# insitro/FastVim

Hardware: AMD Instinct MI355X
Metric: images/sec FastVim-T 224px bs=128/GPU fwd+bwd (+all-reduce +AdamW +EMA), whole job (higher is better)
Workload: dtype bf16; 1 GPU; FastVim-T 224x224 bs=128/GPU bf16 training step, synthetic ImageNet tensors (BASELINE configs[1]); global_batch=128, parallelism=dp1, hip_graph=True, optimizer_in_step=True, final_loss_hex=0x1.779ca20000000p+0

## Files before the change

### fastvim_amd/_lib.py

```python
import ctypes
import os
import threading

import torch

_PKG = os.path.dirname(os.path.abspath(__file__))
LIB_PATH = os.path.join(_PKG, "libfastvim_hip.so")

FV_F32, FV_BF16, FV_F16 = 0, 1, 2
_DTYPES = {torch.float32: FV_F32, torch.bfloat16: FV_BF16, torch.float16: FV_F16}

_lib = None

C_ABI_SYMBOLS = (
    "fv_last_error", "fv_version",
    "fv_selective_scan_fwd", "fv_selective_scan_bwd_workspace", "fv_selective_scan_bwd",
    "fv_causal_conv1d_fwd", "fv_causal_conv1d_bwd", "fv_scan_expand_skip_fwd",
    "fv_mixer_conv_pool_fwd", "fv_mixer_scan_fwd", "fv_mixer_xproj_scan_fwd_ok", "fv_mixer_xproj_scan_fwd", "fv_mixer_combine_fwd",
    "fv_mixer_bwd_blocks", "fv_mixer_combine_bwd", "fv_mixer_scan_bwd_chunks", "fv_mixer_scan_bwd_chunks_b",
    "fv_mixer_scan_bwd_ckpt_floats", "fv_mixer_scan_bwd_partials", "fv_mixer_scan_bwd", "fv_mixer_scan_bwd_dir", "fv_mixer_scan_bwd_ckpt", "fv_mixer_scan_bwd_segments", "fv_mixer_scan_bwd_seg_floats", "fv_mixer_scan_bwd_seg_partials", "fv_mixer_scan_bwd_seg_chunks", "fv_mixer_scan_bwd_seg", "fv_mixer_scan_fwd_ckpt", "fv_mixer_scan_ckpt_floats", "fv_mixer_scan_fwd_segments", "fv_mixer_scan_fwd_seg_floats", "fv_mixer_scan_fwd_seg", "fv_rows_segment_sum", "fv_rows_gather", "fv_mixer_conv_pool_bwd", "fv_mixer_conv_pool_bwd2_ok", "fv_mixer_conv_pool_bwd2", "fv_mixer_scan_bwd_xproj_ok", "fv_mixer_scan_bwd_xproj", "fv_chunk_rows_bf16", "fv_reduce_partials", "fv_reduce_partials_multi",
    "fv_add_norm_blocks", "fv_add_norm_fwd", "fv_add_norm_bwd", "fv_gemm_bf16", "fv_gemm_bf16_tn_grouped", "fv_gemm_bf16_tn_grouped_ld", "fv_mixer_xproj_fwd", "fv_mixer_xproj_bwd_slices", "fv_mixer_xproj_bwd", "fv_mixer_xproj_bwd2", "fv_mixer_xproj_bwd3_ok", "fv_mixer_xproj_bwd3", "fv_adamw_flat", "fv_soft_target_ce",
    "fv_patch_unfold", "fv_gemm_bf16_rowbias", "fv_mean_pool_fwd", "fv_mean_pool_bwd", "fv_droppath_table", "fv_scale_cast",
    "fv_column_sum", "fv_gemm_bf16_addnorm", "fv_gemm_bf16_dgrad_addnorm_blocks", "fv_gemm_bf16_dgrad_addnorm_bwd", "fv_gemm_bf16_dgrad_addnorm_bwd2", "fv_gemm_bf16_addnorm2", "fv_mixer_combine_out_proj_addnorm_ok", "fv_mixer_combine_out_proj_addnorm", "fv_gemm_f32",
    "fv_mixer_conv_pool_bwd_dgrad_ok", "fv_mixer_conv_pool_bwd_dgrad_blocks", "fv_mixer_conv_pool_bwd_dgrad", "fv_transpose_bf16_batched", "fv_gemm_bf16_tn_grouped_wide8",
    "fv_grad_sumsq_blocks", "fv_grad_sumsq_partials", "fv_adamw_flat_groups",
    "fv_pack_weight_frags_batched", "fv_mixer_conv_pool_bwd_dgrad_pk", "fv_mixer_combine_out_proj_addnorm_pk",
    "fv_mix_batch", "fv_patch_unfold_mix", "fv_mixup_target", "fv_label_ce",
    "fv_patch_unfold_chan", "fv_chan_embed_table", "fv_chan_embed_scatter",
)


_tls = threading.local()


class _DeviceGuarded:

    def __init__(self, cdll):
        self._cdll = cdll
        self._wrapped = {}

    def __getattr__(self, name):
        w = self._wrapped.get(name)
        if w is None:
            fn = getattr(self._cdll, name)

            def call(*args, _fn=fn):
                dev = getattr(_tls, "dev", None)
                if dev is None or dev == torch.cuda.current_device():
                    return _fn(*args)
                with torch.cuda.device(dev):
                    return _fn(*args)

            w = self._wrapped[name] = call
        return w


def lib():
    global _lib
    if _lib is None:
        if not os.path.exists(LIB_PATH):
            raise RuntimeError(
                f"{LIB_PATH} is missing: build it with `python -m fastvim_amd.build` "
                "(or __graft_entry__.build()). fastvim_amd has no CPU / eager fallback.")
        cdll = ctypes.CDLL(LIB_PATH)
        cdll.fv_last_error.restype = ctypes.c_char_p
        cdll.fv_selective_scan_bwd_workspace.restype = ctypes.c_size_t
        cdll.fv_mixer_scan_bwd_ckpt_floats.restype = ctypes.c_size_t
        cdll.fv_mixer_scan_ckpt_floats.restype = ctypes.c_size_t
        cdll.fv_mixer_scan_fwd_seg_floats.restype = ctypes.c_size_t
        cdll.fv_mixer_scan_bwd_seg_floats.restype = ctypes.c_size_t
        _lib = _DeviceGuarded(cdll)
    return _lib


def dtype_code(dt):
    try:
        return _DTYPES[dt]
    except KeyError:
        raise RuntimeError(f"fastvim_amd: unsupported dtype {dt}") from None
# ... 26 lines not shown
```

### fastvim_amd/csrc/combine_gemm.hip

```cpp
#include "mixer_common.h"
#include "packed.h"

namespace {

typedef __bf16 cg_bf16x8 __attribute__((ext_vector_type(8)));
typedef float cg_f32x4 __attribute__((ext_vector_type(4)));

constexpr int CG_K = 384, CG_N = 192, CG_BM = 64, CG_NT = 256;
constexpr int CG_RSA = CG_K * 2 + 16;
constexpr int CG_RSB = CG_N * 2 + 16;
constexpr int CG_PD = 6;
constexpr int CG_KS = CG_K / 32;
#ifndef CG_FORCE_PK
#define CG_FORCE_PK 0
#endif
#ifndef CG_DBG
#define CG_DBG 0
#endif

struct CgParams {
  const void* xz;
  const void* skip;
  const float* yc;
  const float *lnw, *lnb;
  void* g;
  float *mean, *rstd_ln;
  float ln_eps;
  Geo geo;
  int B;
  const bf16_t* W;
  long ldw;
  const float* residual;
  const float* nw;
  const float* row_scale;
  int rows_per_scale;
  float* res_out;
  bf16_t* y;
  float* rstd;
  float eps;
  int M;
  int d_in;
};

__device__ __forceinline__ float cg_hsum(f2 v) { return v.x + v.y; }

template <bool PK>
__global__ __launch_bounds__(CG_NT, 2) void combine_out_proj_addnorm_kernel(CgParams p) {
  extern __shared__ __attribute__((aligned(16))) char smem[];
  typedef PairVec<bf16_t, 3> P;
  const int tid = threadIdx.x, lane = tid & 63;
  const int wv = __builtin_amdgcn_readfirstlane(tid >> 6);
  const Geo g = p.geo;
  const int tiles = (g.rows + 3) / 4;
  const int bimg = blockIdx.x / tiles, i0 = (blockIdx.x - bimg * tiles) * 4;
  const int mimg = bimg * g.L;
  auto tok_of = [&](int rl) {
    const int w = rl >> 4, j = rl & 15;
    return (i0 + w < g.rows && j < g.cols) ? mimg + (i0 + w) * g.s_i + j * g.s_j : -1;
  };

  const int lr = lane % 16, gr = lane / 16;
  const int fn = lane & 15, fk = lane >> 4;
  const bf16_t* wrow[3];
  cg_bf16x8 fb[CG_PD][3];
  const char* wpk = reinterpret_cast<const char*>(p.W) + wv * (CG_KS * 3 * 1024);
  const uint32_t wpk_lane = (uint32_t)lane * 16;
  auto wfrag = [&](int nb, int ks) {
    if constexpr (PK) return *reinterpret_cast<const cg_bf16x8*>(wpk + (ks * 3 + nb) * 1024 + wpk_lane);
    else return *reinterpret_cast<const cg_bf16x8*>(wrow[nb] + ks * 32);
  };
  float4 ne_r[2][2][3], ne_w[3];
  float ne_sc[2][2];
  {
#pragma clang fp reassociate(off) contract(off)
    const int lc = lane * 6, voff = lc * 2;
    const int tok_x = 2 * CG_K * 2, tok_s = CG_K * 2;
    const bool has_ln = p.lnw != nullptr;
    const float inv_d = 1.f / (float)p.d_in;
    const size_t ydir = (size_t)p.B * g.rows * CG_K;
    const __amdgpu_buffer_rsrc_t bz = fv_make_buf((const bf16_t*)p.xz + CG_K, (size_t)p.M * tok_x - tok_s);
    const __amdgpu_buffer_rsrc_t bs = fv_make_buf(p.skip, (size_t)p.M * tok_s);
    const __amdgpu_buffer_rsrc_t bg = fv_make_buf(p.g, (size_t)p.M * tok_s);
    const __amdgpu_buffer_rsrc_t bmean = fv_make_buf(has_ln ? (const void*)p.mean : p.g, has_ln ? (size_t)p.M * 4 : 0);
    const __amdgpu_buffer_rsrc_t brstd = fv_make_buf(has_ln ? (const void*)p.rstd_ln : p.g, has_ln ? (size_t)p.M * 4 : 0);
    const int irow = i0 + wv;
    const bool wlive = irow < g.rows;
    const int irc = wlive ? irow : g.rows - 1;
    const int mbase = mimg + irc * g.s_i;
    char* arow = smem + (wv * 16) * CG_RSA + lane * 12;
    constexpr int TT = 2;
    const int npair = (g.cols + TT - 1) / TT;
    f2 ysum[3], ysf[3], ysb[3];
    {
      const float* yr = p.yc + ((size_t)bimg * g.rows + irc) * CG_K + lc;
#pragma unroll
      for (int q = 0; q < 3; ++q) {
        ysf[q] = *reinterpret_cast<const f2*>(yr + 2 * q);
        ysb[q] = *reinterpret_cast<const f2*>(yr + ydir + 2 * q);
      }
    }
    struct Pre { P sk[TT], z[TT]; };
    Pre pa, pb;
    auto fetch = [&](Pre& r, int j0) {
#pragma unroll
      for (int t = 0; t < TT; ++t) {
        const int m = mbase + min(j0 + t, g.cols - 1) * g.s_j;
        r.sk[t].load(bs, voff, m * tok_s);
        r.z[t].load(bz, voff, m * tok_x);
      }
    };
    fetch(pa, 0);
    fetch(pb, TT);
    __builtin_amdgcn_sched_barrier(0);
    f2 lw[3], lb[3];
    {
      const float* lwp = has_ln ? p.lnw : p.yc;
      const float* lbp = has_ln ? p.lnb : p.yc;
#pragma unroll
      for (int q = 0; q < 3; ++q) {
        lw[q] = *reinterpret_cast<const f2*>(lwp + lc + 2 * q);
        lb[q] = *reinterpret_cast<const f2*>(lbp + lc + 2 * q);
      }
    }
    __builtin_amdgcn_sched_barrier(0);
#pragma unroll
    for (int nb = 0; nb < 3; ++nb) wrow[nb] = PK ? nullptr : p.W + (long)(wv * 48 + nb * 16 + fn) * p.ldw + fk * 8;
#pragma unroll
    for (int s = 0; s < CG_PD; s += 2)
#pragma unroll
      for (int nb = 0; nb < 3; ++nb)
#pragma unroll
        for (int h = 0; h < 2; ++h) fb[s + h][nb] = wfrag(nb, s + h);
    __builtin_amdgcn_sched_barrier(0);
#pragma unroll
    for (int q = 0; q < 3; ++q) ysum[q] = ysf[q] + ysb[q];
    auto process = [&](Pre& r, int j0) {
      f2 o[TT][3], z[TT][3];
      float s1[TT], mean[TT], rstd[TT];
#pragma unroll
// ... 184 lines not shown
      for (int k = 0; k < 3; ++k) {
        const int c = (k * LPR + lr) * 4;
        float o[4];
#pragma unroll
        for (int e = 0; e < 4; ++e) {
          float t = v[u][k][e] * rstd;
          asm volatile("" : "+v"(t));
          o[e] = t * w[k][e];
        }
        uint2 pk = {pack_bf16x2(o[0], o[1]), pack_bf16x2(o[2], o[3])};
        if (live) *reinterpret_cast<uint2*>(p.y + base + c) = pk;
      }
    }
  }
}

}

extern "C" int fv_mixer_combine_out_proj_addnorm_ok(int batch, int rows, int cols, int tokens_per_patch, int d_inner,
                                                    int d_model, int dtype) {
  return dtype == FV_BF16 && d_inner == CG_K && d_model == CG_N && tokens_per_patch == 1 && batch > 0 && rows > 0 &&
         cols > 0 && cols <= 16 && (long)batch * rows * cols * CG_K * 4 < 0x7fffffffL;
}

static int cg_launch(bool packed, const void* xz, const void* skip, const float* yc, const float* ln_w,
                                                 const float* ln_b, float ln_eps, void* g, float* mean, float* rstd_ln,
                                                 int batch, int rows, int cols, int tok_stride_row, int tok_stride_col,
                                                 const void* W, long ldw, const float* residual,
                                                 const float* norm_weight, const float* row_scale, int rows_per_scale,
                                                 void* y, float* residual_out, float* rstd, float eps,
                                                 fv_stream_t stream) {
  FV_CHECK(xz && skip && yc && g && W && residual && norm_weight && y && residual_out && rstd,
           "mixer_combine_out_proj_addnorm: null pointer");
  FV_CHECK(!ln_w || (ln_b && mean && rstd_ln), "mixer_combine_out_proj_addnorm: LayerNorm needs weight, bias, mean, rstd");
  FV_CHECK(fv_mixer_combine_out_proj_addnorm_ok(batch, rows, cols, 1, CG_K, CG_N, FV_BF16),
           "mixer_combine_out_proj_addnorm: shape not built (fv_mixer_combine_out_proj_addnorm_ok)");
  FV_CHECK((tok_stride_row == cols && tok_stride_col == 1) || (tok_stride_row == 1 && tok_stride_col == rows),
           "mixer_combine_out_proj_addnorm: token strides (%d,%d) are neither row-major nor transposed for a %dx%d grid",
           tok_stride_row, tok_stride_col, rows, cols);
  FV_CHECK(((uintptr_t)W & 15) == 0 && ldw % 8 == 0 && ldw >= CG_K, "mixer_combine_out_proj_addnorm: weight rows must be 16-byte aligned");
  FV_CHECK(!packed || ldw == CG_K, "mixer_combine_out_proj_addnorm_pk: the packed weight has no row padding (ldw = %d)", CG_K);
  FV_CHECK(((uintptr_t)residual & 15) == 0 && ((uintptr_t)residual_out & 15) == 0 && ((uintptr_t)y & 7) == 0 &&
               ((uintptr_t)norm_weight & 15) == 0, "mixer_combine_out_proj_addnorm: row operands must be 16-byte aligned");
  FV_CHECK(!row_scale || rows_per_scale > 0, "mixer_combine_out_proj_addnorm: rows_per_scale must be positive");
  CgParams p{};
  p.xz = xz; p.skip = skip; p.yc = yc; p.lnw = ln_w; p.lnb = ln_b; p.g = g; p.mean = mean; p.rstd_ln = rstd_ln;
  p.ln_eps = ln_eps;
  p.geo = make_geo(rows, cols, tok_stride_row, tok_stride_col, 1);
  p.B = batch;
  p.W = (const bf16_t*)W; p.ldw = ldw; p.residual = residual; p.nw = norm_weight; p.row_scale = row_scale;
  p.rows_per_scale = rows_per_scale; p.res_out = residual_out; p.y = (bf16_t*)y; p.rstd = rstd; p.eps = eps;
  p.M = batch * rows * cols;
  p.d_in = CG_K;
  const size_t smem = (size_t)CG_BM * CG_RSA;
  const dim3 grid(batch * fv_cdiv(rows, 4)), block(CG_NT);
  if (packed || CG_FORCE_PK) hipLaunchKernelGGL(combine_out_proj_addnorm_kernel<true>, grid, block, smem, (hipStream_t)stream, p);
  else hipLaunchKernelGGL(combine_out_proj_addnorm_kernel<false>, grid, block, smem, (hipStream_t)stream, p);
  FV_LAUNCH_CHECK();
  return FV_OK;
}

#define CG_ARGS_DECL                                                                                                          \
  const void *xz, const void *skip, const float *yc, const float *ln_w, const float *ln_b, float ln_eps, void *g,             \
      float *mean, float *rstd_ln, int batch, int rows, int cols, int tok_stride_row, int tok_stride_col, const void *W,      \
      long ldw, const float *residual, const float *norm_weight, const float *row_scale, int rows_per_scale, void *y,         \
      float *residual_out, float *rstd, float eps, fv_stream_t stream
#define CG_ARGS                                                                                                               \
  xz, skip, yc, ln_w, ln_b, ln_eps, g, mean, rstd_ln, batch, rows, cols, tok_stride_row, tok_stride_col, W, ldw, residual,    \
      norm_weight, row_scale, rows_per_scale, y, residual_out, rstd, eps, stream

extern "C" int fv_mixer_combine_out_proj_addnorm(CG_ARGS_DECL) { return cg_launch(false, CG_ARGS); }

extern "C" int fv_mixer_combine_out_proj_addnorm_pk(CG_ARGS_DECL) { return cg_launch(true, CG_ARGS); }
```

### fastvim_amd/csrc/convpool_dgrad.hip

```cpp
#include "mixer_common.h"
#include "packed.h"
#include "gemm_tiles.h"

namespace {

constexpr int CD_DI = 384, CD_N = 192, CD_K = 2 * CD_DI, CD_BM = 64, CD_NT = 256, CD_NCH = CD_DI / 128;
constexpr int CD_RSA = CD_DI * 2 + 16;
constexpr int CD_RSB = CD_N * 2 + 16;
#ifndef CD_PDEPTH
#define CD_PDEPTH 4
#endif
#ifndef CD_SB_EVERY
#define CD_SB_EVERY 1
#endif
#ifndef CD_W2_PIPE
#define CD_W2_PIPE 1
#endif
constexpr int CD_PD = CD_PDEPTH;
constexpr int CD_KS = CD_K / 32;
constexpr int CD_ZST = CD_BM * BK * 2;
constexpr int CD_NZ = CD_DI / BK;
constexpr int CD_O_RING = CD_BM * CD_RSA;
constexpr int CD_SLOT = 12 * 128;
constexpr int CD_O_B = (CD_BM * CD_RSB + 255) / 256 * 256, CD_O_S = CD_O_B + 2 * 128 * BK * 2;
constexpr int CD_SMEM = CD_O_S + 4 * 32 * (64 * 2 + 16);
static_assert(CD_O_RING + 3 * CD_ZST <= CD_SMEM && CD_O_RING + 4 * CD_SLOT * 4 <= CD_SMEM, "LDS regions");
static_assert(2 * CD_SMEM <= 160 * 1024, "two workgroups per CU");
#ifndef CD_FORCE_PK
#define CD_FORCE_PK 0
#endif
#ifndef CD_DBG
#define CD_DBG 0
#endif

struct CdParams {
  const void* xz;
  const void* dob;
  const float* dxc;
  const void* dxc2;
  const float *wf, *bf, *wb, *bb, *Df, *Db;
  void* dxz;
  float* part;
  float pool_scale;
  Geo geo;
  int B;
  const bf16_t* Wt;
  long ldwt;
  const float* dres_out;
  const float* r;
  const float* rstd;
  const float* nw;
  const float* row_scale;
  int rows_per_scale;
  bf16_t* dx;
  float* dres_in;
  float* pw;
  const bf16_t* W2;
  long ldw2;
  bf16_t* C2;
  int N2;
  int M;
};

__device__ __forceinline__ void cd_dma16(const void* base, uint32_t voff, uint32_t lds_dst) {
  asm volatile("s_mov_b32 m0, %2\n\ts_nop 0\n\tglobal_load_lds_dwordx4 %0, %1" ::"v"(voff), "s"(base), "s"(lds_dst) : "memory");
}

constexpr int cd_younger(int t) {
  constexpr int KX = CD_DI / 32;
  int n = 0;
  for (int q = KX + 2 * (t - 3) + 2; q < KX + 2 * t; q += 2) n += (q + CD_PD < CD_KS ? 6 : 0) + ((q - KX) / 2 + 3 < CD_NZ ? 2 : 0);
  return n;
}
static_assert(cd_younger(3) < 64 && cd_younger(4) < 64 && cd_younger(5) < 64, "vmcnt is a 6-bit counter");

template <int NT, bool X2, bool PK>
__global__ __launch_bounds__(CD_NT, 2) void conv_pool_bwd_dgrad_kernel(CdParams p) {
  extern __shared__ __attribute__((aligned(16))) char smem[];
  typedef PairVec<bf16_t, 1> P;
  const int tid = threadIdx.x, lane = tid & 63;
  const int wv = __builtin_amdgcn_readfirstlane(tid >> 6);
  const Geo g = p.geo;
  const int tiles = (g.rows + 3) / 4;
  const int bimg = blockIdx.x / tiles, i0 = (blockIdx.x - bimg * tiles) * 4;
  const int mimg = bimg * g.L;
  auto tok_of = [&](int rl) {
    const int w = rl >> 4, j = rl & 15;
    return (i0 + w < g.rows && j < g.cols) ? mimg + (i0 + w) * g.s_i + j * g.s_j : -1;
  };
  const int irow = i0 + wv;
  const bool wlive = irow < g.rows;
  char* prow = smem + (wv * 16) * CD_RSA;

  {
    const int zr0 = wlive ? NT : 0;
    for (int e = lane; e < (16 - zr0) * (CD_RSA / 4); e += 64) reinterpret_cast<uint32_t*>(prow + zr0 * CD_RSA)[e] = 0u;
    const int tok_x = 2 * CD_DI * 2, tok_d = CD_DI * 2;
    const size_t dstride = (size_t)p.B * g.rows * CD_DI;
    const __amdgpu_buffer_rsrc_t bp = fv_make_buf(p.dxc, 2 * dstride * 4);
    const __amdgpu_buffer_rsrc_t bp2 = fv_make_buf(X2 ? p.dxc2 : p.dxc, X2 ? 2 * dstride * 2 : 0);
    const int irc = wlive ? irow : 0;
    const bool up = irc > 0, down = irc + 1 < g.rows;
    const int m_row = irc * g.s_i, s_up = up ? -g.s_i : 0, s_dn = down ? g.s_i : 0;
    const int pooled_off = (bimg * g.rows + irc) * CD_DI;
    const size_t img_x = (size_t)bimg * g.L * 2 * CD_DI, img_d = (size_t)bimg * g.L * CD_DI;
    const __amdgpu_buffer_rsrc_t bx = fv_make_buf((const bf16_t*)p.xz + img_x, wlive ? (size_t)g.L * tok_x : 0);
    const __amdgpu_buffer_rsrc_t bd = fv_make_buf((const bf16_t*)p.dob + img_d, wlive ? (size_t)g.L * tok_d : 0);
    const __amdgpu_buffer_rsrc_t bo = fv_make_buf((bf16_t*)p.dxz + img_x, wlive ? (size_t)g.L * tok_x : 0);
    struct Pooled {
      f2 a;
      P b;
      __device__ __forceinline__ f2 sum() const { if constexpr (X2) return a + b.get(0); else return a; }
    };
    auto pooled = [&](int r, bool backward, int c0, bool on) {
      const bool ok = r == 1 || (r == 0 ? up : down);
      uint32_t w[2];
      const int eoff = pooled_off + (ok ? (r - 1) * CD_DI : 0) + (backward ? (int)dstride : 0);
      const int lane_off = on ? c0 : 0x1ffffff0;
      fv_buf_load_words<2>(bp, lane_off * 4, eoff * 4, w);
      Pooled o;
      o.a.x = __uint_as_float(w[0]);
      o.a.y = __uint_as_float(w[1]);
      if constexpr (X2) o.b.load(bp2, lane_off * 2, eoff * 2);
      return o;
    };
    P xr[NT + 6], dr[NT + 6];
    auto fetch = [&](int k, int voff) {
      const int di = k < 3 ? -1 : (k >= NT + 3 ? 1 : 0);
      const int j = k - 3 - di * NT;
      const int m = m_row + (di < 0 ? s_up : di > 0 ? s_dn : 0) + j * g.s_j;
      xr[k].load(bx, voff, m * tok_x);
      dr[k].load(bd, voff, m * tok_d);
    };
    struct Prm { f2 wf[CW], wb[CW], bf, bb, Df, Db; };
    auto load_prm = [&](int c0) {
      Prm q;
      load_taps2(p.wf, c0, q.wf);
      load_taps2(p.wb, c0, q.wb);
      q.bf = load_f2(p.bf ? p.bf : p.wf, c0);
      q.bb = load_f2(p.bb ? p.bb : p.wf, c0);
      q.Df = load_f2(p.Df ? p.Df : p.wf, c0);
      q.Db = load_f2(p.Db ? p.Db : p.wf, c0);
      return q;
    };
// ... 51 lines not shown
            pf = fma2(wf[k], x[k0 + k], pf);
            pb = fma2(wb[k], x[k3 - k], pb);
          }
          const f2 sgf = sigmoid2(pf), sgb = sigmoid2(pb);
          const f2 dsf = sgf * fma2(pf, 1.f - sgf, splat(1.f)), dsb = sgb * fma2(pb, 1.f - sgb, splat(1.f));
          const float e3 = q3 < NT ? 1.f : m_dn, e0 = n >= 0 ? 1.f : m_up;
          if (q3 == NT) cf_dn = cf_dn_raw.sum() * (down ? p.pool_scale : 0.f);
          const f2 nf = fma2(Dfh, dov[k3], q3 >= NT ? cf_dn : cf_mid) * dsf * e3;
          const f2 nb = fma2(Dbh, dov[k0], n < 0 ? cb_up : cb_mid) * dsb * e0;
          if (n == -1) cb_up_raw = pooled(0, true, c0n, more);
          dpf[k3] = nf;
          dpb[k0] = nb;
          if (q3 < NT) {
#pragma unroll
            for (int k = 0; k < CW; ++k) a_wf[k] = fma2(nf, x[k0 + k], a_wf[k]);
            a_bf += nf;
            a_Df = fma2(dov[k3], pf * sgf, a_Df);
          }
          if (n >= 0) {
#pragma unroll
            for (int k = 0; k < CW; ++k) a_wb[k] = fma2(nb, x[k3 - k], a_wb[k]);
            a_bb += nb;
            a_Db = fma2(dov[k0], pb * sgb, a_Db);
            f2 dx = splat(0.f);
#pragma unroll
            for (int k = 0; k < CW; ++k) {
              dx = fma2(wf[k], dpf[k3 - k], dx);
              dx = fma2(wb[k], dpb[k0 - 3 + k], dx);
            }
            const uint32_t pk[1] = {pack_bf16x2(dx.x, dx.y)};
            fv_buf_store_words<1>(bo, voff, (m_row + n * g.s_j) * tok_x, pk);
            *reinterpret_cast<uint32_t*>(prow + n * CD_RSA + voff) = pk[0];
          }
          if ((n + 3) % CD_SB_EVERY == CD_SB_EVERY - 1) __builtin_amdgcn_sched_barrier(0);
        }
        cf_dn_raw = pooled(2, false, c0n, more);
      }
      {
        const f2 hDf = a_Df * 0.5f, hDb = a_Db * 0.5f;
        float4* s4 = reinterpret_cast<float4*>(slot);
        s4[2 * lane] = make_float4(a_wf[0].x, a_wf[1].x, a_wf[2].x, a_wf[3].x);
        s4[2 * lane + 1] = make_float4(a_wf[0].y, a_wf[1].y, a_wf[2].y, a_wf[3].y);
        s4[128 + 2 * lane] = make_float4(a_wb[0].x, a_wb[1].x, a_wb[2].x, a_wb[3].x);
        s4[128 + 2 * lane + 1] = make_float4(a_wb[0].y, a_wb[1].y, a_wb[2].y, a_wb[3].y);
        f2* s2 = reinterpret_cast<f2*>(slot + 1024);
        s2[lane] = a_bf;
        s2[64 + lane] = a_bb;
        s2[128 + lane] = hDf;
        s2[192 + lane] = hDb;
      }
      __syncthreads();
      {
        const float* s0 = reinterpret_cast<const float*>(smem + CD_O_RING);
        float* dst = p.part + (size_t)blockIdx.x * 12 * CD_DI;
#pragma unroll
        for (int i = 0; i < CD_SLOT / CD_NT; ++i) {
          const int e = tid + i * CD_NT;
          const float v = ((s0[e] + s0[CD_SLOT + e]) + s0[2 * CD_SLOT + e]) + s0[3 * CD_SLOT + e];
          int gi;
          if (e < 512) gi = c * 512 + e;
          else if (e < 1024) gi = 4 * CD_DI + c * 512 + (e - 512);
          else {
            const int q = (e - 1024) >> 7, rr = (e - 1024) & 127;
            gi = (8 + q) * CD_DI + c * 128 + rr;
          }
          dst[gi] = v;
        }
      }
      __syncthreads();
    }
  }

  const int fn = lane & 15, fk = lane >> 4, lr = lane % 16, gr = lane / 16;
  const bf16_t* wrow[3];
  bf16x8 fb[CD_PD][3];
#pragma unroll
  for (int nb = 0; nb < 3; ++nb) wrow[nb] = PK ? nullptr : p.Wt + (long)(wv * 48 + nb * 16 + fn) * p.ldwt + fk * 8;
  const char* wpk = reinterpret_cast<const char*>(p.Wt) + wv * (CD_KS * 3 * 1024);
  const uint32_t wpk_lane = (uint32_t)lane * 16;
  auto wfrag = [&](int nb, int ks) {
    if constexpr (PK) return *reinterpret_cast<const bf16x8*>(wpk + (ks * 3 + nb) * 1024 + wpk_lane);
    else return *reinterpret_cast<const bf16x8*>(wrow[nb] + ks * 32);
  };
  uint32_t zoff[2];
  const uint32_t ring = (uint32_t)(uintptr_t)(__attribute__((address_space(3))) const char*)(smem + CD_O_RING);
#pragma unroll
  for (int i = 0; i < 2; ++i) {
    const int e = tid + i * CD_NT, rrow = e >> 3, ch = (e & 7) ^ (rrow & 7);
    const int m = tok_of(rrow);
    zoff[i] = (uint32_t)((m >= 0 ? m : mimg) * (CD_K * 2) + (CD_DI + ch * 8) * 2);
  }
  auto issue_z = [&](int t) {
#pragma unroll
    for (int i = 0; i < 2; ++i)
      cd_dma16(p.dxz, zoff[i] + (uint32_t)t * (BK * 2), ring + (uint32_t)(t % 3) * CD_ZST + (uint32_t)(i * CD_NT + wv * 64) * 16);
  };
  issue_z(0);
  issue_z(1);
  issue_z(2);
#pragma unroll
  for (int s = 0; s < CD_PD; s += 2)
#pragma unroll
    for (int nb = 0; nb < 3; ++nb)
#pragma unroll
      for (int h = 0; h < 2; ++h) fb[s + h][nb] = wfrag(nb, s + h);
  __builtin_amdgcn_sched_barrier(0);
  float4 ne_r[2][2][3];
// ... 121 lines not shown
#pragma unroll
          for (int e = 0; e < 4; ++e) {
            const float dyl = dyv[e] * lv;
            xh[k][e] = (rr[e] - 0.f) * rstd;
            dxh[k][e] = dyl * w[k][e];
            aw[k][e] = fmaf(dyl, xh[k][e], aw[k][e]);
            c2 = fmaf(dxh[k][e], xh[k][e], c2);
          }
        }
#define FV_DPP_ADD(ctrl) c2 += __int_as_float(__builtin_amdgcn_update_dpp(0, __float_as_int(c2), ctrl, 0xf, 0xf, true))
        FV_DPP_ADD(0xB1);
        FV_DPP_ADD(0x4E);
        FV_DPP_ADD(0x141);
        FV_DPP_ADD(0x140);
#undef FV_DPP_ADD
        c2 = c2 * inv_n;
        const float c1 = 0.f;
#pragma unroll
        for (int k = 0; k < 3; ++k) {
          const int c = (k * LPR + lr) * 4;
          const float4 g4 = ne_g[it][u][k];
          const float gg[4] = {g4.x, g4.y, g4.z, g4.w};
          float dr[4];
#pragma unroll
          for (int e = 0; e < 4; ++e) dr[e] = rstd * (dxh[k][e] - c1 - xh[k][e] * c2) + gg[e];
          if (live) {
            *reinterpret_cast<float4*>(p.dres_in + base + c) = make_float4(dr[0], dr[1], dr[2], dr[3]);
            if (p.row_scale)
#pragma unroll
              for (int e = 0; e < 4; ++e) dr[e] *= sc;
            uint2 pk = {pack_bf16x2(dr[0], dr[1]), pack_bf16x2(dr[2], dr[3])};
            *reinterpret_cast<uint2*>(p.dx + base + c) = pk;
            *reinterpret_cast<uint2*>(smem + rl * CD_RSB + c * 2) = pk;
          } else {
            *reinterpret_cast<uint2*>(smem + rl * CD_RSB + c * 2) = make_uint2(0u, 0u);
          }
        }
      }
    }
    __syncthreads();
    float* s_acc = reinterpret_cast<float*>(smem + CD_BM * CD_RSB);
#pragma unroll
    for (int k = 0; k < 3; ++k)
#pragma unroll
      for (int e = 0; e < 4; ++e) {
        float v = aw[k][e];
        auto r1 = __builtin_amdgcn_permlane16_swap(__float_as_uint(v), __float_as_uint(v), false, false);
        v = __uint_as_float(r1[0]) + __uint_as_float(r1[1]);
        auto r2 = __builtin_amdgcn_permlane32_swap(__float_as_uint(v), __float_as_uint(v), false, false);
        v = __uint_as_float(r2[0]) + __uint_as_float(r2[1]);
        if (gr == 0) s_acc[wv * CD_N + (k * LPR + lr) * 4 + e] = v;
      }
    __syncthreads();
    float* dst = p.pw + (size_t)blockIdx.x * CD_N;
    for (int c = tid; c < CD_N; c += CD_NT) dst[c] = (s_acc[c] + s_acc[CD_N + c]) + (s_acc[2 * CD_N + c] + s_acc[3 * CD_N + c]);
  }
  if (p.W2 && CD_DBG != 4) {
    __syncthreads();
    tile_times_w2_rows<CD_BM, CD_RSB, KS, decltype(tok_of), CD_W2_PIPE != 0>(smem, smem + CD_O_B, smem + CD_O_S, p.W2, p.ldw2, p.N2,
                                                                              p.C2, tok_of, tid);
  }
}

}

extern "C" int fv_mixer_conv_pool_bwd_dgrad_ok(int batch, int rows, int cols, int tokens_per_patch, int d_inner, int d_model,
                                               int pool_max, int dtype) {
  return dtype == FV_BF16 && d_inner == CD_DI && d_model == CD_N && tokens_per_patch == 1 && !pool_max && batch > 0 &&
         rows > 0 && (cols == 14 || cols == 16) &&
         (long)batch * rows * cols * CD_K * 2 < 0x7fffffffL &&
         (long)batch * rows * CD_DI * 8 < 0x7ffff000L;
}

extern "C" int fv_mixer_conv_pool_bwd_dgrad_blocks(int batch, int rows) { return batch * fv_cdiv(rows, 4); }

static int cd_launch(
    bool packed, const void* xz, const void* dskip, const float* dxc, const void* dxc2, const float* conv_w, const float* conv_b,
    const float* conv_w_b, const float* conv_b_b, const float* D, const float* D_b, void* dxz, float* conv_partials, int batch,
    int rows, int cols, int tok_stride_row, int tok_stride_col, float scaling, const void* W_in_t, long ldwt,
    const float* dresidual_out, const float* r, const float* rstd, const float* norm_weight, const float* row_scale,
    int rows_per_scale, void* dx, float* dresidual_in, float* partial_dw, const void* W2, void* C2, int N2, long ldw2,
    fv_stream_t stream) {
  FV_CHECK(xz && dskip && dxc && conv_w && conv_w_b && dxz && conv_partials && W_in_t && r && rstd && norm_weight && dx &&
               dresidual_in && partial_dw, "mixer_conv_pool_bwd_dgrad: null pointer");
  FV_CHECK(fv_mixer_conv_pool_bwd_dgrad_ok(batch, rows, cols, 1, CD_DI, CD_N, 0, FV_BF16),
           "mixer_conv_pool_bwd_dgrad: shape not built (fv_mixer_conv_pool_bwd_dgrad_ok)");
  FV_CHECK((tok_stride_row == cols && tok_stride_col == 1) || (tok_stride_row == 1 && tok_stride_col == rows),
           "mixer_conv_pool_bwd_dgrad: token strides (%d,%d) are neither row-major nor transposed for a %dx%d grid",
           tok_stride_row, tok_stride_col, rows, cols);
  FV_CHECK(((uintptr_t)W_in_t & 15) == 0 && ldwt % 8 == 0 && ldwt >= CD_K, "mixer_conv_pool_bwd_dgrad: transposed weight rows must be 16-byte aligned");
  FV_CHECK(!packed || ldwt == CD_K, "mixer_conv_pool_bwd_dgrad_pk: the packed weight has no row padding (ldwt = %d)", CD_K);
  FV_CHECK(((uintptr_t)r & 15) == 0 && ((uintptr_t)dresidual_in & 15) == 0 && ((uintptr_t)dx & 7) == 0 &&
               ((uintptr_t)norm_weight & 15) == 0 && ((uintptr_t)dresidual_out & 15) == 0 && ((uintptr_t)dxz & 15) == 0,
           "mixer_conv_pool_bwd_dgrad: row operands must be 16-byte aligned");
  FV_CHECK(!row_scale || rows_per_scale > 0, "mixer_conv_pool_bwd_dgrad: rows_per_scale must be positive");
  FV_CHECK(!W2 || (C2 && N2 > 0 && N2 % 128 == 0 && ldw2 % 8 == 0 && ldw2 >= N2 && ((uintptr_t)W2 & 15) == 0 && ((uintptr_t)C2 & 15) == 0),
           "mixer_conv_pool_bwd_dgrad: the second weight must be (192, N2) with N2 a multiple of 128, 16-byte aligned");
  CdParams p{};
  p.xz = xz; p.dob = dskip; p.dxc = dxc; p.dxc2 = dxc2; p.wf = conv_w; p.bf = conv_b; p.wb = conv_w_b; p.bb = conv_b_b;
  p.Df = D; p.Db = D_b; p.dxz = dxz; p.part = conv_partials;
  p.pool_scale = scaling / (float)cols;
  p.geo = make_geo(rows, cols, tok_stride_row, tok_stride_col, 1);
  p.B = batch;
  p.Wt = (const bf16_t*)W_in_t; p.ldwt = ldwt; p.dres_out = dresidual_out; p.r = r; p.rstd = rstd; p.nw = norm_weight;
  p.row_scale = row_scale; p.rows_per_scale = rows_per_scale > 0 ? rows_per_scale : 1; p.dx = (bf16_t*)dx;
  p.dres_in = dresidual_in; p.pw = partial_dw; p.W2 = (const bf16_t*)W2; p.ldw2 = ldw2; p.C2 = (bf16_t*)C2; p.N2 = N2;
  p.M = batch * rows * cols;
  const dim3 grid(batch * fv_cdiv(rows, 4)), block(CD_NT);
#define FV_CD(NTT, XX, PP)                                                                                          \
  do {                                                                                                              \
    static FvOncePerDevice done;                                                                                    \
    if (done.first())                                                                                               \
      (void)hipFuncSetAttribute((const void*)conv_pool_bwd_dgrad_kernel<NTT, XX, PP>, hipFuncAttributeMaxDynamicSharedMemorySize, CD_SMEM); \
    hipLaunchKernelGGL((conv_pool_bwd_dgrad_kernel<NTT, XX, PP>), grid, block, CD_SMEM, (hipStream_t)stream, p);    \
  } while (0)
#define FV_CD2(NTT, XX) do { if (packed || CD_FORCE_PK) FV_CD(NTT, XX, true); else FV_CD(NTT, XX, false); } while (0)
  if (cols == 14) { if (dxc2) FV_CD2(14, true); else FV_CD2(14, false); }
  else { if (dxc2) FV_CD2(16, true); else FV_CD2(16, false); }
#undef FV_CD2
#undef FV_CD
  FV_LAUNCH_CHECK();
  return FV_OK;
}

#define CD_ARGS_DECL                                                                                                          \
  const void *xz, const void *dskip, const float *dxc, const void *dxc2, const float *conv_w, const float *conv_b,            \
      const float *conv_w_b, const float *conv_b_b, const float *D, const float *D_b, void *dxz, float *conv_partials,        \
      int batch, int rows, int cols, int tok_stride_row, int tok_stride_col, float scaling, const void *W_in_t, long ldwt,    \
      const float *dresidual_out, const float *r, const float *rstd, const float *norm_weight, const float *row_scale,        \
      int rows_per_scale, void *dx, float *dresidual_in, float *partial_dw, const void *W2, void *C2, int N2, long ldw2,      \
      fv_stream_t stream
#define CD_ARGS                                                                                                               \
  xz, dskip, dxc, dxc2, conv_w, conv_b, conv_w_b, conv_b_b, D, D_b, dxz, conv_partials, batch, rows, cols, tok_stride_row,    \
      tok_stride_col, scaling, W_in_t, ldwt, dresidual_out, r, rstd, norm_weight, row_scale, rows_per_scale, dx,              \
      dresidual_in, partial_dw, W2, C2, N2, ldw2, stream

extern "C" int fv_mixer_conv_pool_bwd_dgrad(CD_ARGS_DECL) { return cd_launch(false, CD_ARGS); }

extern "C" int fv_mixer_conv_pool_bwd_dgrad_pk(CD_ARGS_DECL) { return cd_launch(true, CD_ARGS); }
```

### include/fastvim_hip.h

```cpp
#ifndef FASTVIM_HIP_H
#define FASTVIM_HIP_H

#include <stddef.h>
#include <stdint.h>

#ifdef __cplusplus
extern "C" {
#endif

typedef void* fv_stream_t;

enum { FV_F32 = 0, FV_BF16 = 1, FV_F16 = 2 };
enum { FV_OK = 0, FV_ERR_INVALID = -1, FV_ERR_HIP = -2, FV_ERR_UNSUPPORTED = -3 };

const char* fv_last_error(void);
#define FV_ABI_VERSION 3
int fv_version(void);

int fv_selective_scan_fwd(const void* u, const void* delta, const float* A, const void* B,
                          const void* C, const float* D, const void* z, const float* delta_bias,
                          void* out, float* last_state, int batch, int dim, int seqlen, int dstate,
                          int n_groups, int B_variable, int C_variable, int delta_softplus,
                          int dtype, fv_stream_t stream);

// ... 118 lines not shown

int fv_add_norm_blocks(int M);
int fv_add_norm_fwd(const void* x, int x_dtype, const void* residual, int residual_dtype,
                    const float* weight, const float* bias, const float* row_scale, int rows_per_scale,
                    void* y, int y_dtype, void* residual_out, int residual_out_dtype, float* mean,
                    float* rstd, int M, int N, float eps, int is_rms_norm, fv_stream_t stream);
int fv_add_norm_bwd(const void* dy, int dy_dtype, const void* dresidual_out, int dresidual_out_dtype,
                    const void* r, int r_dtype, const float* weight, const float* mean, const float* rstd,
                    const float* row_scale, int rows_per_scale, void* dx, int dx_dtype, void* dresidual_in,
                    int dresidual_in_dtype, float* partial_dw, float* partial_db, int M, int N,
                    int is_rms_norm, fv_stream_t stream);

int fv_gemm_bf16(const void* A, const void* B, void* C, const float* bias, int M, int N, int K, long lda,
                 long ldb, long ldc, int a_k_slow, int b_k_slow, int c_fp32, int splits, fv_stream_t stream);

int fv_gemm_f32(const void* A, int a_dtype, const void* B, int b_dtype, void* C, int c_dtype, const float* bias, int M,
                int N, int K, long lda, long ldb, long ldc, int a_k_slow, int b_k_slow, int batch, long strideA,
                long strideB, long strideC, fv_stream_t stream);

int fv_gemm_bf16_addnorm(const void* A, const void* W, const float* residual, const float* norm_weight,
                         const float* row_scale, int rows_per_scale, void* y, float* residual_out, float* rstd, int M,
                         int N, int K, long lda, long ldw, float eps, fv_stream_t stream);

int fv_gemm_bf16_dgrad_addnorm_blocks(int M);
int fv_gemm_bf16_dgrad_addnorm_bwd(const void* A, const void* W, const float* dresidual_out, const float* r,
                                   const float* rstd, const float* norm_weight, const float* row_scale,
                                   int rows_per_scale, void* dx, float* dresidual_in, float* partial_dw, int M, int N,
                                   int K, long lda, long ldw, fv_stream_t stream);

int fv_gemm_bf16_dgrad_addnorm_bwd2(const void* A, const void* W, const float* dresidual_out, const float* r,
                                    const float* rstd, const float* norm_weight, const float* row_scale,
                                    int rows_per_scale, void* dx, float* dresidual_in, float* partial_dw, int M, int N,
                                    int K, long lda, long ldw, const void* W2, void* C2, int N2, long ldw2,
                                    fv_stream_t stream);

int fv_mixer_combine_out_proj_addnorm_ok(int batch, int rows, int cols, int tokens_per_patch, int d_inner, int d_model,
                                         int dtype);
int fv_mixer_combine_out_proj_addnorm(const void* xz, const void* skip, const float* yc, const float* ln_w,
                                      const float* ln_b, float ln_eps, void* g, float* mean, float* rstd_ln, int batch,
                                      int rows, int cols, int tok_stride_row, int tok_stride_col, const void* W, long ldw,
                                      const float* residual, const float* norm_weight, const float* row_scale,
                                      int rows_per_scale, void* y, float* residual_out, float* rstd, float eps,
                                      fv_stream_t stream);
int fv_mixer_combine_out_proj_addnorm_pk(const void* xz, const void* skip, const float* yc, const float* ln_w,
                                         const float* ln_b, float ln_eps, void* g, float* mean, float* rstd_ln, int batch,
                                         int rows, int cols, int tok_stride_row, int tok_stride_col, const void* W,
                                         long ldw, const float* residual, const float* norm_weight,
                                         const float* row_scale, int rows_per_scale, void* y, float* residual_out,
                                         float* rstd, float eps, fv_stream_t stream);

int fv_mixer_conv_pool_bwd_dgrad_ok(int batch, int rows, int cols, int tokens_per_patch, int d_inner, int d_model,
                                    int pool_max, int dtype);
int fv_mixer_conv_pool_bwd_dgrad_blocks(int batch, int rows);
int fv_mixer_conv_pool_bwd_dgrad(const void* xz, const void* dskip, const float* dxc, const void* dxc2,
                                 const float* conv_w, const float* conv_b, const float* conv_w_b, const float* conv_b_b,
                                 const float* D, const float* D_b, void* dxz, float* conv_partials, int batch, int rows,
                                 int cols, int tok_stride_row, int tok_stride_col, float scaling, const void* W_in_t,
                                 long ldwt, const float* dresidual_out, const float* r, const float* rstd,
                                 const float* norm_weight, const float* row_scale, int rows_per_scale, void* dx,
                                 float* dresidual_in, float* partial_dw, const void* W2, void* C2, int N2, long ldw2,
                                 fv_stream_t stream);
int fv_mixer_conv_pool_bwd_dgrad_pk(const void* xz, const void* dskip, const float* dxc, const void* dxc2,
                                    const float* conv_w, const float* conv_b, const float* conv_w_b,
                                    const float* conv_b_b, const float* D, const float* D_b, void* dxz,
                                    float* conv_partials, int batch, int rows, int cols, int tok_stride_row,
                                    int tok_stride_col, float scaling, const void* W_in_t, long ldwt,
                                    const float* dresidual_out, const float* r, const float* rstd,
                                    const float* norm_weight, const float* row_scale, int rows_per_scale, void* dx,
                                    float* dresidual_in, float* partial_dw, const void* W2, void* C2, int N2, long ldw2,
                                    fv_stream_t stream);

int fv_transpose_bf16_batched(const void* const* srcs, void* const* dsts, int njobs, int rows, int cols,
                              fv_stream_t stream);

int fv_pack_weight_frags_batched(const void* const* srcs, void* const* dsts, int njobs, int K, fv_stream_t stream);

int fv_gemm_bf16_addnorm2(const void* A, const void* W, const float* residual, const float* norm_weight,
                          const float* row_scale, int rows_per_scale, void* y, float* residual_out, float* rstd, int M,
                          int N, int K, long lda, long ldw, float eps, const void* W2, void* C2, int N2, long ldw2,
                          fv_stream_t stream);

int fv_gemm_bf16_tn_grouped(const void* const* x, const void* const* y, float* const* parts, const int* Kd,
                            const int* M, const int* N, const int* splits, int count, fv_stream_t stream);
int fv_gemm_bf16_tn_grouped_ld(const void* const* x, const void* const* y, float* const* parts, const int* Kd,
                               const int* M, const int* N, const int* ldx, const int* ldy, const int* splits, int count,
                               fv_stream_t stream);

int fv_gemm_bf16_tn_grouped_wide8(int M, int N, int Kd);

int fv_mixer_xproj_fwd(const void* xc, const void* x_proj_w2, void* x_dbl, int M, int d_inner, int width,
                       fv_stream_t stream);

int fv_mixer_xproj_bwd_slices(int M);
int fv_mixer_xproj_bwd(const float* dx_dbl_partials, int nchunks, const void* xc, const float* x_proj_w,
                       const float* x_proj_w_b, float* dxc, float* dW_partials, int M, int d_inner, int width,
                       int dtype, fv_stream_t stream);
int fv_mixer_xproj_bwd2(const float* dx_dbl_partials, int nchunks, const void* xc, const float* x_proj_w,
                        const float* x_proj_w_b, float* dxc, float* dW_partials, void* dx_dbl_bf16, int M, int d_inner,
                        int width, int dtype, fv_stream_t stream);
int fv_mixer_xproj_bwd3_ok(int M, int d_inner, int width, int dtype);
int fv_mixer_xproj_bwd3(const float* dx_dbl_partials, int nchunks, const void* xc, const float* x_proj_w,
                        const float* x_proj_w_b, const void* x_proj_w_t_bf16, float* dxc, void* dxc2_bf16,
                        void* dx_dbl_bf16, int M, int d_inner, int width, int dtype, fv_stream_t stream);

int fv_soft_target_ce(const void* logits, int logits_dtype, const float* target, float* loss_rows, float* loss,
                      float* dlogits, int batch, int classes, fv_stream_t stream);
// ... 55 lines not shown
```

Measured before the change: 25880 images/sec.

## Remap fused mixer tiles: XCD-contiguous image-major order with balanced row heights

The fused combine/out_proj and conv-pool dgrad kernels now map block IDs through a shared tile function. It assigns contiguous tile ranges to each of the 8 XCDs (blocks round-robin across XCDs) so neighbouring rows of an image share an L2. It also spreads rows evenly across tiles, so no tile is a ragged 4-row-minus remainder. Partial outputs are indexed by the logical tile id, so downstream reductions stay consistent. Optional tuning hooks and timestamp probes are compiled only under a macro, and the change adds a little index arithmetic per block.

```diff
diff --git a/fastvim_amd/_lib.py b/fastvim_amd/_lib.py
--- a/fastvim_amd/_lib.py
+++ b/fastvim_amd/_lib.py
@@ -25,6 +25,7 @@
     "fv_mixer_conv_pool_bwd_dgrad_ok", "fv_mixer_conv_pool_bwd_dgrad_blocks", "fv_mixer_conv_pool_bwd_dgrad", "fv_transpose_bf16_batched", "fv_gemm_bf16_tn_grouped_wide8",
     "fv_grad_sumsq_blocks", "fv_grad_sumsq_partials", "fv_adamw_flat_groups",
     "fv_pack_weight_frags_batched", "fv_mixer_conv_pool_bwd_dgrad_pk", "fv_mixer_combine_out_proj_addnorm_pk",
+    "fv_mixer_fused_tile",
     "fv_mix_batch", "fv_patch_unfold_mix", "fv_mixup_target", "fv_label_ce",
     "fv_patch_unfold_chan", "fv_chan_embed_table", "fv_chan_embed_scatter",
 )
diff --git a/fastvim_amd/csrc/combine_gemm.hip b/fastvim_amd/csrc/combine_gemm.hip
--- a/fastvim_amd/csrc/combine_gemm.hip
+++ b/fastvim_amd/csrc/combine_gemm.hip
@@ -1,5 +1,6 @@
 #include "mixer_common.h"
 #include "packed.h"
+#include "fused_tiles.h"
 
 namespace {
 
@@ -40,6 +41,9 @@
   float eps;
   int M;
   int d_in;
+#ifdef FASTVIM_TUNING_HOOKS
+  int tile_order;
+#endif
 };
 
 __device__ __forceinline__ float cg_hsum(f2 v) { return v.x + v.y; }
@@ -51,12 +55,17 @@
   const int tid = threadIdx.x, lane = tid & 63;
   const int wv = __builtin_amdgcn_readfirstlane(tid >> 6);
   const Geo g = p.geo;
-  const int tiles = (g.rows + 3) / 4;
-  const int bimg = blockIdx.x / tiles, i0 = (blockIdx.x - bimg * tiles) * 4;
+#ifdef FASTVIM_TUNING_HOOKS
+  const int tile_order = p.tile_order;
+#else
+  constexpr int tile_order = FV_TILES_ORDER;
+#endif
+  const FvFusedTile tile = fv_fused_tile_of(p.B, g.rows, (int)blockIdx.x, tile_order);
+  const int bimg = tile.image, i0 = tile.row0, th = tile.height;
   const int mimg = bimg * g.L;
   auto tok_of = [&](int rl) {
     const int w = rl >> 4, j = rl & 15;
-    return (i0 + w < g.rows && j < g.cols) ? mimg + (i0 + w) * g.s_i + j * g.s_j : -1;
+    return (w < th && j < g.cols) ? mimg + (i0 + w) * g.s_i + j * g.s_j : -1;
   };
 
   const int lr = lane % 16, gr = lane / 16;
@@ -84,7 +93,7 @@
     const __amdgpu_buffer_rsrc_t bmean = fv_make_buf(has_ln ? (const void*)p.mean : p.g, has_ln ? (size_t)p.M * 4 : 0);
     const __amdgpu_buffer_rsrc_t brstd = fv_make_buf(has_ln ? (const void*)p.rstd_ln : p.g, has_ln ? (size_t)p.M * 4 : 0);
     const int irow = i0 + wv;
-    const bool wlive = irow < g.rows;
+    const bool wlive = wv < th;
     const int irc = wlive ? irow : g.rows - 1;
     const int mbase = mimg + irc * g.s_i;
     char* arow = smem + (wv * 16) * CG_RSA + lane * 12;
@@ -375,6 +384,9 @@
   p.rows_per_scale = rows_per_scale; p.res_out = residual_out; p.y = (bf16_t*)y; p.rstd = rstd; p.eps = eps;
   p.M = batch * rows * cols;
   p.d_in = CG_K;
+#ifdef FASTVIM_TUNING_HOOKS
+  p.tile_order = fv_tune("FASTVIM_FUSED_TILES", FV_TILES_ORDER);
+#endif
   const size_t smem = (size_t)CG_BM * CG_RSA;
   const dim3 grid(batch * fv_cdiv(rows, 4)), block(CG_NT);
   if (packed || CG_FORCE_PK) hipLaunchKernelGGL(combine_out_proj_addnorm_kernel<true>, grid, block, smem, (hipStream_t)stream, p);
diff --git a/fastvim_amd/csrc/convpool_dgrad.hip b/fastvim_amd/csrc/convpool_dgrad.hip
--- a/fastvim_amd/csrc/convpool_dgrad.hip
+++ b/fastvim_amd/csrc/convpool_dgrad.hip
@@ -1,6 +1,7 @@
 #include "mixer_common.h"
 #include "packed.h"
 #include "gemm_tiles.h"
+#include "fused_tiles.h"
 
 namespace {
 
@@ -60,7 +61,37 @@
   bf16_t* C2;
   int N2;
   int M;
+#ifdef FASTVIM_TUNING_HOOKS
+  int tile_order;
+  unsigned long long* stamps;
+#endif
 };
+
+#ifdef FASTVIM_TUNING_HOOKS
+extern "C" unsigned long long* fv_debug_get_stamps();
+__device__ __forceinline__ void cd_stamp_time(const CdParams& p, int slot) {
+  if (p.stamps && threadIdx.x == 0) {
+    __builtin_amdgcn_sched_barrier(0);
+    const unsigned long long t = __builtin_amdgcn_s_memrealtime();
+    __builtin_amdgcn_sched_barrier(0);
+    p.stamps[(size_t)blockIdx.x * 8 + slot] = t;
+  }
+}
+__device__ __forceinline__ void cd_stamp_place(const CdParams& p, int id, int height) {
+  if (p.stamps && threadIdx.x == 0) {
+    unsigned long long* s = p.stamps + (size_t)blockIdx.x * 8;
+    s[2] = __builtin_amdgcn_s_getreg((20 << 0) | (0 << 6) | (3 << 11)) & 0xf;
+    s[3] = (unsigned)__builtin_amdgcn_s_getreg((4 << 0) | (0 << 6) | (31 << 11));
+    s[4] = id;
+    s[5] = height;
+  }
+}
+#define CD_STAMP_TIME(slot) cd_stamp_time(p, slot)
+#define CD_STAMP_PLACE(id, h) cd_stamp_place(p, id, h)
+#else
+#define CD_STAMP_TIME(slot) ((void)0)
+#define CD_STAMP_PLACE(id, h) ((void)0)
+#endif
 
 __device__ __forceinline__ void cd_dma16(const void* base, uint32_t voff, uint32_t lds_dst) {
   asm volatile("s_mov_b32 m0, %2\n\ts_nop 0\n\tglobal_load_lds_dwordx4 %0, %1" ::"v"(voff), "s"(base), "s"(lds_dst) : "memory");
@@ -81,15 +112,22 @@
   const int tid = threadIdx.x, lane = tid & 63;
   const int wv = __builtin_amdgcn_readfirstlane(tid >> 6);
   const Geo g = p.geo;
-  const int tiles = (g.rows + 3) / 4;
-  const int bimg = blockIdx.x / tiles, i0 = (blockIdx.x - bimg * tiles) * 4;
+#ifdef FASTVIM_TUNING_HOOKS
+  const int tile_order = p.tile_order;
+#else
+  constexpr int tile_order = FV_TILES_ORDER;
+#endif
+  const FvFusedTile tile = fv_fused_tile_of(p.B, g.rows, (int)blockIdx.x, tile_order);
+  const int bimg = tile.image, i0 = tile.row0, th = tile.height;
   const int mimg = bimg * g.L;
+  CD_STAMP_TIME(0);
+  CD_STAMP_PLACE(tile.id, th);
   auto tok_of = [&](int rl) {
     const int w = rl >> 4, j = rl & 15;
-    return (i0 + w < g.rows && j < g.cols) ? mimg + (i0 + w) * g.s_i + j * g.s_j : -1;
+    return (w < th && j < g.cols) ? mimg + (i0 + w) * g.s_i + j * g.s_j : -1;
   };
   const int irow = i0 + wv;
-  const bool wlive = irow < g.rows;
+  const bool wlive = wv < th;
   char* prow = smem + (wv * 16) * CD_RSA;
 
   {
@@ -247,7 +285,7 @@
       __syncthreads();
       {
         const float* s0 = reinterpret_cast<const float*>(smem + CD_O_RING);
-        float* dst = p.part + (size_t)blockIdx.x * 12 * CD_DI;
+        float* dst = p.part + (size_t)tile.id * 12 * CD_DI;
 #pragma unroll
         for (int i = 0; i < CD_SLOT / CD_NT; ++i) {
           const int e = tid + i * CD_NT;
@@ -475,7 +513,7 @@
         if (gr == 0) s_acc[wv * CD_N + (k * LPR + lr) * 4 + e] = v;
       }
     __syncthreads();
-    float* dst = p.pw + (size_t)blockIdx.x * CD_N;
+    float* dst = p.pw + (size_t)tile.id * CD_N;
     for (int c = tid; c < CD_N; c += CD_NT) dst[c] = (s_acc[c] + s_acc[CD_N + c]) + (s_acc[2 * CD_N + c] + s_acc[3 * CD_N + c]);
   }
   if (p.W2 && CD_DBG != 4) {
@@ -483,6 +521,7 @@
     tile_times_w2_rows<CD_BM, CD_RSB, KS, decltype(tok_of), CD_W2_PIPE != 0>(smem, smem + CD_O_B, smem + CD_O_S, p.W2, p.ldw2, p.N2,
                                                                               p.C2, tok_of, tid);
   }
+  CD_STAMP_TIME(1);
 }
 
 }
@@ -496,6 +535,15 @@
 }
 
 extern "C" int fv_mixer_conv_pool_bwd_dgrad_blocks(int batch, int rows) { return batch * fv_cdiv(rows, 4); }
+
+extern "C" int fv_mixer_fused_tile(int batch, int rows, int hw_block, int* image, int* row0, int* height) {
+  if (batch <= 0 || rows <= 0 || hw_block < 0 || (long)hw_block >= (long)batch * fv_cdiv(rows, 4)) return -1;
+  const FvFusedTile t = fv_fused_tile_of(batch, rows, hw_block, fv_tune("FASTVIM_FUSED_TILES", FV_TILES_ORDER));
+  if (image) *image = t.image;
+  if (row0) *row0 = t.row0;
+  if (height) *height = t.height;
+  return t.id;
+}
 
 static int cd_launch(
     bool packed, const void* xz, const void* dskip, const float* dxc, const void* dxc2, const float* conv_w, const float* conv_b,
@@ -529,6 +577,10 @@
   p.row_scale = row_scale; p.rows_per_scale = rows_per_scale > 0 ? rows_per_scale : 1; p.dx = (bf16_t*)dx;
   p.dres_in = dresidual_in; p.pw = partial_dw; p.W2 = (const bf16_t*)W2; p.ldw2 = ldw2; p.C2 = (bf16_t*)C2; p.N2 = N2;
   p.M = batch * rows * cols;
+#ifdef FASTVIM_TUNING_HOOKS
+  p.tile_order = fv_tune("FASTVIM_FUSED_TILES", FV_TILES_ORDER);
+  p.stamps = fv_debug_get_stamps();
+#endif
   const dim3 grid(batch * fv_cdiv(rows, 4)), block(CD_NT);
 #define FV_CD(NTT, XX, PP)                                                                                          \
   do {                                                                                                              \
diff --git a/fastvim_amd/csrc/fused_tiles.h b/fastvim_amd/csrc/fused_tiles.h
--- /dev/null
+++ b/fastvim_amd/csrc/fused_tiles.h
@@ -0,0 +1,55 @@
+#pragma once
+
+#if defined(__HIPCC__) || defined(__CUDACC__)
+#define FV_TILES_HD __host__ __device__
+#else
+#define FV_TILES_HD
+#endif
+
+enum { FV_TILES_IMAGE_MAJOR = 0, FV_TILES_TALL_FIRST = 1, FV_TILES_LEGACY = 2 };
+#ifndef FV_TILES_ORDER
+#define FV_TILES_ORDER FV_TILES_IMAGE_MAJOR
+#endif
+
+struct FvFusedTile {
+  int id;
+  int image;
+  int row0;
+  int height;
+};
+
+FV_TILES_HD inline FvFusedTile fv_fused_tile_of(int batch, int rows, int hw_block, int order) {
+  const int tiles = (rows + 3) / 4, nblk = batch * tiles;
+  FvFusedTile o;
+  if (order == FV_TILES_LEGACY) {
+    o.id = hw_block;
+    o.image = hw_block / tiles;
+    o.row0 = (hw_block - o.image * tiles) * 4;
+    o.height = rows - o.row0 < 4 ? rows - o.row0 : 4;
+    return o;
+  }
+  const int base = rows / tiles, extra = rows % tiles;
+  const int q8 = nblk / 8, r8 = nblk % 8, xcd = hw_block % 8, j = hw_block / 8;
+  const int s = xcd < r8 ? xcd * (q8 + 1) : r8 * (q8 + 1) + (xcd - r8) * q8;
+  int id = s + j;
+  if (order == FV_TILES_TALL_FIRST && extra != 0) {
+    const int n = q8 + (xcd < r8 ? 1 : 0), e = s + n;
+    const int ms = s % tiles, me = e % tiles;
+    const int t0 = (s / tiles) * extra + (ms < extra ? ms : extra);
+    const int t1 = (e / tiles) * extra + (me < extra ? me : extra);
+    const int ntall = t1 - t0, shorts = tiles - extra;
+    if (j < ntall) {
+      const int k = t0 + j;
+      id = (k / extra) * tiles + k % extra;
+    } else {
+      const int k = (s - t0) + (j - ntall);
+      id = (k / shorts) * tiles + extra + k % shorts;
+    }
+  }
+  const int image = id / tiles, t = id - image * tiles;
+  o.id = id;
+  o.image = image;
+  o.row0 = t * base + (t < extra ? t : extra);
+  o.height = base + (t < extra ? 1 : 0);
+  return o;
+}
diff --git a/include/fastvim_hip.h b/include/fastvim_hip.h
--- a/include/fastvim_hip.h
+++ b/include/fastvim_hip.h
@@ -194,6 +194,7 @@
 int fv_mixer_conv_pool_bwd_dgrad_ok(int batch, int rows, int cols, int tokens_per_patch, int d_inner, int d_model,
                                     int pool_max, int dtype);
 int fv_mixer_conv_pool_bwd_dgrad_blocks(int batch, int rows);
+int fv_mixer_fused_tile(int batch, int rows, int hw_block, int* image, int* row0, int* height);
 int fv_mixer_conv_pool_bwd_dgrad(const void* xz, const void* dskip, const float* dxc, const void* dxc2,
                                  const float* conv_w, const float* conv_b, const float* conv_w_b, const float* conv_b_b,
                                  const float* D, const float* D_b, void* dxz, float* conv_partials, int batch, int rows,
```

New measurement: 25830 images/sec. No clear change (-0.2%).
